# werner-duvaud/muzero-general

Measured on NVIDIA H100. Metric: self-play env-steps/sec, higher is better.
Workload: dtype f32 nets + f64 tree statistics

## Files before the change

muzero_general_b200/csrc/fc_search.cu:

```cuda
#include "fc_net.cuh"
#include "tree.cuh"
#include "kernels.h"

#include <stdlib.h>
#include <algorithm>
#include <vector>

namespace mz {

struct GameSmem {
    int vsum, mval, root_prior, visit, expansion, reward, prior, path, path_reward, hidden, act, bytes;
};

__host__ __device__ inline GameSmem game_smem_layout(int N, int A, int E, int maxw, bool keep_hidden) {
    GameSmem L;
    const int S = (N + 1) * A;
    const int Epad = (E + 3) & ~3;
    int off = 0;
    auto take = [&](int bytes) { int o = off; off = (off + bytes + 15) & ~15; return o; };
    L.vsum = take(S * 8);
    L.mval = take(S * 8);
    L.root_prior = take(A * 8);
    L.visit = take(S * 4);
    L.expansion = take(S * 4);
    L.reward = take(S * 4);
    L.prior = take(S * 4);
    L.path = take((N + 2) * 4);
    L.path_reward = take((N + 2) * 4);
    L.hidden = take((keep_hidden ? (N + 1) * Epad : 0) * 4);
    L.act = take(9 * maxw * 4);
    off += 16;
    L.bytes = off;
    return L;
}

enum { kPhRoot, kPhSelect, kPhNet, kPhExpand, kPhBackup, kPhLevels, kPhRounds, kPhSims, kPhSums,
       kPhStart = kPhSums, kPhEnd, kPhCount };
#ifdef MZ_FC_PHASES
constexpr int kPhMaxGames = 1 << 16;
__device__ unsigned long long g_fc_phase[kPhMaxGames][kPhCount];
MZ_DEVINL unsigned long long global_ns() {
    unsigned long long t;
    asm volatile("mov.u64 %0, %%globaltimer;" : "=l"(t));
    return t;
}
struct PhaseClock {
    int row = -1;
    unsigned last = 0;
    MZ_DEVINL void start(int g, bool leader) {
        row = (leader && g < kPhMaxGames) ? g : -1;
        if (row >= 0) atomicExch(&g_fc_phase[row][kPhStart], global_ns());
        last = (unsigned)clock();
    }
    MZ_DEVINL void finish() { if (row >= 0) atomicExch(&g_fc_phase[row][kPhEnd], global_ns()); }
    MZ_DEVINL void mark(int p) {
        const unsigned now = (unsigned)clock();
        if (row >= 0) atomicAdd(&g_fc_phase[row][p], (unsigned long long)(now - last));
        last = now;
    }
    MZ_DEVINL void count(int p, int n) { if (row >= 0) atomicAdd(&g_fc_phase[row][p], (unsigned long long)n); }
};
#else
struct PhaseClock {
    MZ_DEVINL void start(int, bool) {}
    MZ_DEVINL void finish() {}
    MZ_DEVINL void mark(int) {}
    MZ_DEVINL void count(int, int) {}
};
#endif

enum { kTapRaw, kTapReward, kTapPolicy, kTapValue };
struct NoTap { MZ_DEVINL void operator()(int, const float*, int) const {} };

template <int G, typename Tap>
MZ_DEVINL void fc_root_inference(const FcNet& net, const float* blob, const float* obs, float* hidden, float* s0, float* s1,
                                 float* s2, int E, int S, int A, float& logit, float& value, Tap&& tap) {
    const int lane = LaneGroup<G>::lane();
    load_vector<G>(obs, s1, net.obs_elems);
    float* raw = mlp_forward<G>(net.rep, blob, s1, s0, s1, s2);
    tap(kTapRaw, raw, E);
    rescale_unit_range<G>(raw, hidden, E);
    float* pol = mlp_forward<G>(net.pol, blob, hidden, s0, s1, s2);
    logit = (lane < A) ? pol[lane] : 0.0f;
    tap(kTapPolicy, pol, A);
    LaneGroup<G>::sync();
    float* val = mlp_forward<G>(net.val, blob, hidden, s0, s1, s2);
    value = support_to_scalar_group<G>(val, S);
    tap(kTapValue, val, 2 * S + 1);
    LaneGroup<G>::sync();
}

template <int G, typename SH, typename Tap>
MZ_DEVINL void fc_sim_inference(const FcNet& net, const float* blob, const float* h, int action, float* hn, float* s0, float* s1,
                                float* s2, float* const (&hb)[3][2], bool fused_heads, int E, int S, int A, float& logit,
                                float& prior, float& value, float& reward, Tap&& tap) {
    const int lane = LaneGroup<G>::lane();
    const int F = 2 * S + 1;
    if constexpr (SH::kEnabled) {
        fc_recurrent_fixed<G, SH>(net, blob, h, action, hn, s0, s1, hb[0][0], hb[1][0], hb[2][0], prior, value, reward);
        tap(kTapRaw, s1, E);
    } else {
        float* raw = mlp_forward<G>(net.dyn, blob, h, s0, s1, s2, action);
        if (fused_heads) {
            rescale_unit_range<G>(raw, hn, E);
            const MlpDesc* const ds[3] = {&net.rew, &net.pol, &net.val};
            const float* const xs[3] = {raw, hn, hn};
            float* outs[3];
            mlp_forward_multi<G, 3>(ds, blob, xs, hb, outs);
            logit = (lane < A) ? outs[1][lane] : 0.0f;
            support_to_scalar_group2<G>(outs[2], outs[0], S, value, reward);
            tap(kTapRaw, raw, E); tap(kTapReward, outs[0], F); tap(kTapPolicy, outs[1], A); tap(kTapValue, outs[2], F);
            LaneGroup<G>::sync();
        } else {
            float* rl = mlp_forward<G>(net.rew, blob, raw, s0, s1, nullptr);
            reward = support_to_scalar_group<G>(rl, S);
            tap(kTapRaw, raw, E); tap(kTapReward, rl, F);
            LaneGroup<G>::sync();
            rescale_unit_range<G>(raw, hn, E);
            float* pol = mlp_forward<G>(net.pol, blob, hn, s0, s1, s2);
            logit = (lane < A) ? pol[lane] : 0.0f;
            tap(kTapPolicy, pol, A);
            LaneGroup<G>::sync();
            float* vl = mlp_forward<G>(net.val, blob, hn, s0, s1, s2);
            value = support_to_scalar_group<G>(vl, S);
            tap(kTapValue, vl, F);
            LaneGroup<G>::sync();
        }
        prior = group_softmax_masked<G>(logit, lane < A);
    }
}

template <typename SH>
constexpr int fixed_actions() {
    if constexpr (SH::kEnabled) return SH::A;
    else return 0;
}

template <int G, bool kTeacher, typename SH, int kP>
__global__ void __launch_bounds__(kFcMaxThreads, 2) fc_search_kernel(const __grid_constant__ FcSearchArgs a) {
    extern __shared__ __align__(16) unsigned char smem[];
    constexpr int kA = fixed_actions<SH>();
    const int N = a.N, A = kA ? kA : a.A;
    double* s_pbc = reinterpret_cast<double*>(smem);
    double* s_sqrt = s_pbc + (N + 2);
    float* s_blob = reinterpret_cast<float*>(s_sqrt + (N + 2));
    for (int i = threadIdx.x; i < N + 2; i += blockDim.x) { s_pbc[i] = a.pbc[i]; s_sqrt[i] = a.sqrtn[i]; }
    if (!kTeacher)
        for (int i = threadIdx.x; i < a.net.blob_floats; i += blockDim.x) s_blob[i] = a.blob[i];
    __syncthreads();

    const int shared_bytes = ((2 * (N + 2) * 8 + (kTeacher ? 0 : a.net.blob_floats) * 4) + 15) & ~15;
    const GameSmem L = game_smem_layout(N, A, a.net.E, a.net.maxw, !kTeacher);
    const int groups_per_cta = blockDim.x / G;
    const int gi = threadIdx.x / G;
    const int lane = LaneGroup<G>::lane();
    unsigned char* mine = smem + shared_bytes + (size_t)gi * L.bytes;

    TreeConst c;
    c.A = A; c.N = N; c.P = a.P; c.discount = a.discount; c.noise_frac = a.noise_frac; c.noise_alpha = a.noise_alpha; c.seed = a.seed;
    c.pbc = s_pbc; c.sqrtn = s_sqrt; c.ucb = a.ucb;

    GameTree t;
    t.vsum = reinterpret_cast<double*>(mine + L.vsum);
    t.mval = reinterpret_cast<double*>(mine + L.mval);
    t.root_prior = reinterpret_cast<double*>(mine + L.root_prior);
    t.visit = reinterpret_cast<int*>(mine + L.visit);
    t.expansion = reinterpret_cast<int*>(mine + L.expansion);
    t.reward = reinterpret_cast<float*>(mine + L.reward);
    t.prior = reinterpret_cast<float*>(mine + L.prior);
    t.path = reinterpret_cast<int*>(mine + L.path);
    t.path_reward = reinterpret_cast<float*>(mine + L.path_reward);
    float* s_hidden = reinterpret_cast<float*>(mine + L.hidden);
    float* s_act = reinterpret_cast<float*>(mine + L.act);
    const int E = a.net.E, S = a.net.S, maxw = a.net.maxw;
    const int Epad = (E + 3) & ~3;
    float* s0 = s_act;
    float* s1 = s_act + maxw;
    float* s2 = s_act + 2 * maxw;
    float* const hb[3][2] = {{s_act + 3 * maxw, s_act + 4 * maxw}, {s_act + 5 * maxw, s_act + 6 * maxw},
                             {s_act + 7 * maxw, s_act + 8 * maxw}};
    const bool fused_heads = (a.net.rew.n == a.net.pol.n) && (a.net.pol.n == a.net.val.n);
    constexpr int kMaxD = select_levels_for(kA ? kA : 2, G);
    const SelectLanes sl = select_lanes<G, kA>(A, min(a.select_levels, kMaxD));
    PhaseClock ph;

    const int warp_first = (int)blockIdx.x * groups_per_cta + (int)(threadIdx.x & ~31u) / G;
    for (int g0 = warp_first; g0 < a.n_games; g0 += gridDim.x * groups_per_cta) {
        const int g_own = g0 + gi - (int)(threadIdx.x & ~31u) / G;
        const bool own = g_own < a.n_games;
        const int g = own ? g_own : a.n_games - 1;
        ph.start(g, lane == 0 && own);
        const int64_t game_id = a.game_id ? a.game_id[g] : (int64_t)g;
        const int move = a.move_index ? a.move_index[g] : 0;
        const int to_play0 = a.to_play ? a.to_play[g] : 0;
        const int first_index = a.first_index ? a.first_index[g] : -1;
        unsigned legal = 0;
        for (int k = 0; k < A; ++k) legal |= (a.legal_mask == nullptr || a.legal_mask[(size_t)g * A + k]) ? (1u << k) : 0u;
        t.legal = legal;
        (void)to_play0;

        float root_value, root_reward, logit = 0.0f;
        if (kTeacher) {
            root_value = a.teacher.root_value[g];
            root_reward = a.teacher.root_reward[g];
        } else {
            fc_root_inference<G>(a.net, s_blob, a.obs + (size_t)g * a.net.obs_elems, s_hidden, s0, s1, s2, E, S, A, logit, root_value,
                                 NoTap{});
            root_reward = inverse_value_transform(0.0f);
        }
        float prior;
        if (kTeacher) prior = (lane < A) ? a.teacher.root_priors[(size_t)g * A + lane] : 0.0f;
        else prior = group_softmax_masked<G>(logit, lane < A && ((legal >> lane) & 1u));
        if (a.trace.root_priors_raw && lane < A && own) a.trace.root_priors_raw[(size_t)g * A + lane] = ((legal >> lane) & 1u) ? prior : 0.0f;
        if (a.trace.root_reward && lane == 0 && own) a.trace.root_reward[g] = root_reward;
        tree_init_root<G, kA>(c, t, prior, root_reward,
                              (a.add_noise && a.noise) ? a.noise + (size_t)g * A : nullptr, a.add_noise && !a.noise,
                              game_id, move, (a.trace.noise && own) ? a.trace.noise + (size_t)g * A : nullptr);
        ph.mark(kPhRoot);

        int max_depth = 0;
        LaneGroup<G>::converge();
        for (int sim = 0; sim < N; ++sim) {
            int rounds;
            const Leaf leaf = tree_select_lookahead<G, kMaxD, kA>(c, t, sl, sim, game_id, move, first_index, rounds);
            ph.mark(kPhSelect);
            ph.count(kPhLevels, leaf.depth);
            ph.count(kPhRounds, rounds);
            float value, reward;
            if (kTeacher) {
                value = a.teacher.value[(size_t)g * N + sim];
                reward = a.teacher.reward[(size_t)g * N + sim];
                prior = (lane < A) ? a.teacher.priors[((size_t)g * N + sim) * A + lane] : 0.0f;
            } else {
                fc_sim_inference<G, SH>(a.net, s_blob, s_hidden + (size_t)leaf.parent_exp * Epad, leaf.action,
                                        s_hidden + (size_t)t.n_expanded * Epad, s0, s1, s2, hb, fused_heads, E, S, A, logit, prior, value, reward,
                                        NoTap{});
            }
            ph.mark(kPhNet);
            if (a.trace.depth && own) {
                const size_t ti = (size_t)g * N + sim;
                if (lane == 0) { a.trace.depth[ti] = leaf.depth; a.trace.value[ti] = value; a.trace.reward[ti] = reward; }
                if (lane < A) a.trace.priors[ti * A + lane] = prior;
                for (int j = lane; j < leaf.depth && j < a.trace.max_depth; j += G)
                    a.trace.actions[ti * a.trace.max_depth + j] = (uint8_t)(t.path[j + 1] % A);
            }
            tree_expand<G, kA>(c, t, leaf, reward, prior);
            ph.mark(kPhExpand);
            tree_backup<G, kP, true>(c, t, leaf, value);
            ph.mark(kPhBackup);
            max_depth = max(max_depth, leaf.depth);
        }
        ph.count(kPhSims, N);

        if (lane < A && own) {
            const bool ok = (legal >> lane) & 1u;
            if (a.visit_counts) a.visit_counts[(size_t)g * A + lane] = ok ? t.visit[lane] : 0;
            if (a.root_priors) a.root_priors[(size_t)g * A + lane] = t.root_prior[lane];
        }
        if (lane == 0 && own) {
            if (a.root_value) a.root_value[g] = (t.root_visit == 0) ? 0.0 : __ddiv_rn(t.root_vsum, (double)t.root_visit);
            if (a.root_predicted_value) a.root_predicted_value[g] = root_value;
            if (a.max_tree_depth) a.max_tree_depth[g] = max_depth;
            if (a.tie_count) a.tie_count[g] = t.ties;
            if (a.value_range) { a.value_range[2 * g] = t.lo; a.value_range[2 * g + 1] = t.hi; }
        }
        if (a.pool.visit && own) {
            const int slots = (N + 1) * A;
            const size_t pb = (size_t)g * slots;
            for (int s = lane; s < t.n_expanded * A; s += G) {
                a.pool.visit[pb + s] = t.visit[s];
                a.pool.vsum[pb + s] = t.vsum[s];
                a.pool.reward[pb + s] = t.reward[s];
                a.pool.prior[pb + s] = t.prior[s];
                a.pool.expansion[pb + s] = t.expansion[s];
            }
            if (lane < A) a.pool.root_prior[(size_t)g * A + lane] = t.root_prior[lane];
            if (!kTeacher && a.pool.hidden)
                for (int i = lane; i < t.n_expanded * E; i += G)
                    a.pool.hidden[(size_t)g * (N + 1) * E + i] = s_hidden[(i / E) * Epad + (i % E)];
            if (lane == 0) {
                a.pool.root_visit[g] = t.root_visit;
                a.pool.root_vsum[g] = t.root_vsum;
                a.pool.n_expanded[g] = t.n_expanded;
            }
        }
        ph.finish();
        LaneGroup<G>::sync();
    }
}

static size_t fc_cta_smem(int N, int A, int E, int maxw, int blob_floats, bool teacher, int groups) {
    const GameSmem L = game_smem_layout(N, A, E, maxw, !teacher);
    const size_t shared_bytes = ((2 * (size_t)(N + 2) * 8 + (teacher ? 0 : (size_t)blob_floats) * 4) + 15) & ~(size_t)15;
    return shared_bytes + (size_t)groups * L.bytes;
}

bool fc_search_plan(int N, int A, int E, int maxw, int blob_floats, int G, bool teacher, int n_games, int sm_count,
                    size_t smem_per_sm, size_t smem_reserve, size_t smem_cap, int regs, int threads, FcPlan* plan) {
    if (n_games < 1 || sm_count < 1 || G < 1 || regs < 1 || N < 0 || A < 1 || E < 1 || maxw < 1 || blob_floats < 0) return false;
    bool found = false;
    const std::vector<int> sizes = threads != 0 ? std::vector<int>{threads} : std::vector<int>{64, 128, 256};
    for (int t : sizes) {
        if (t % 32 != 0 || t < G || t > kFcMaxThreads) continue;
        const int groups = t / G;
        const size_t smem = fc_cta_smem(N, A, E, maxw, blob_floats, teacher, groups);
        const int by_smem = smem > smem_cap ? 0 : (int)(smem_per_sm / ((smem + smem_reserve + 127) & ~(size_t)127));
        const int by_regs = (65536 / (((regs * 32) + 255) & ~255)) / (t / 32);
        const int per_sm = std::min(std::min(by_smem, by_regs), std::min(2048 / t, 32));
        if (per_sm >= 1) {
            const int slots = per_sm * groups * sm_count;
            const int passes = (n_games + slots - 1) / slots;
            if (!found || passes < plan->passes) {
                *plan = FcPlan{t, groups, per_sm, slots, passes, smem};
                found = true;
            }
        }
    }
    return found;
}

template <int G, bool T, typename SH, int kP>
static cudaError_t launch_kernel(const FcSearchArgs& a, const FcLaunchInfo& l, cudaStream_t stream) {
    fc_search_kernel<G, T, SH, kP><<<l.grid, l.block, l.smem, stream>>>(a);
    return cudaGetLastError();
}

template <int G, bool T, typename SH, int kP = 0>
static cudaError_t prepare_one(const FcSearchArgs& a, bool one_level, int sm_count, FcLaunchState* st, FcPrepared* p) {
    p->select_levels = one_level ? 1 : select_levels_for(a.A, G);
    auto kern = fc_search_kernel<G, T, SH, kP>;
    const void* fn = reinterpret_cast<const void*>(kern);
    int regs = 0;
    for (const auto& k : st->kernels) if (k.fn == fn) regs = k.regs;
    if (regs == 0) {
        cudaError_t err = cudaFuncSetAttribute(kern, cudaFuncAttributeMaxDynamicSharedMemorySize, (int)st->smem_cap);
        if (err == cudaSuccess) err = cudaFuncSetAttribute(kern, cudaFuncAttributePreferredSharedMemoryCarveout, cudaSharedmemCarveoutMaxShared);
        cudaFuncAttributes fa{};
        if (err == cudaSuccess) err = cudaFuncGetAttributes(&fa, kern);
        if (err != cudaSuccess) return err;
        regs = fa.numRegs;
        st->kernels.push_back({fn, regs});
    }
    FcPlan plan;
    if (!fc_search_plan(a.N, a.A, a.net.E, a.net.maxw, a.net.blob_floats, G, T, a.n_games, sm_count, st->smem_per_sm,
                        st->smem_reserve, st->smem_cap, regs, a.threads, &plan))
        return cudaErrorInvalidConfiguration;
    int per_sm = -1;
    for (const auto& s : st->shapes) if (s.fn == fn && s.threads == plan.threads && s.smem == plan.smem) per_sm = s.ctas_per_sm;
    if (per_sm < 0) {
        cudaError_t err = cudaOccupancyMaxActiveBlocksPerMultiprocessor(&per_sm, kern, plan.threads, plan.smem);
        if (err != cudaSuccess) return err;
        st->shapes.push_back({fn, plan.threads, plan.smem, per_sm});
    }
    per_sm = std::min(per_sm, plan.ctas_per_sm);
    if (per_sm < 1) return cudaErrorInvalidConfiguration;
    const int want = (a.n_games + plan.groups - 1) / plan.groups;
    const int grid = std::min(want, per_sm * sm_count);
    p->launch = launch_kernel<G, T, SH, kP>;
    p->fixed_shape = SH::kEnabled;
    p->info = FcLaunchInfo{grid, plan.threads, per_sm, G, plan.smem};
    return cudaSuccess;
}

using CartPoleShape = FcFixedShape<8, 16, 10, 2>;

static bool fc_uses_fixed(const FcNet& net, int G) { return (G == 16 || G == 32) && fc_matches_fixed<CartPoleShape>(net); }

static cudaError_t prepare_fc_search(const FcSearchArgs& a, int group, bool teacher, bool generic, bool one_level,
                                     int sm_count, FcLaunchState* st, FcPrepared* p) {
    if (!teacher && !generic && fc_uses_fixed(a.net, group)) {
        if (group == 16 && a.P == 1) return prepare_one<16, false, CartPoleShape, 1>(a, one_level, sm_count, st, p);
        if (group == 16) return prepare_one<16, false, CartPoleShape>(a, one_level, sm_count, st, p);
        if (group == 32 && a.P == 1) return prepare_one<32, false, CartPoleShape, 1>(a, one_level, sm_count, st, p);
        if (group == 32) return prepare_one<32, false, CartPoleShape>(a, one_level, sm_count, st, p);
    }
#define MZ_CASE(GG)                                                                                     \
    case GG:                                                                                            \
        return teacher ? prepare_one<GG, true, FcGenericShape>(a, one_level, sm_count, st, p)           \
                       : prepare_one<GG, false, FcGenericShape>(a, one_level, sm_count, st, p);
    switch (group) {
        MZ_CASE(4)
        MZ_CASE(8)
        MZ_CASE(16)
        MZ_CASE(32)
    }
#undef MZ_CASE
    return cudaErrorInvalidValue;
}

cudaError_t launch_fc_search(const FcSearchArgs& a_in, int group, bool teacher, int sm_count, FcLaunchState* st,
                             cudaStream_t stream) {
    const char* generic = getenv("MZ_FC_GENERIC");
    const char* levels = getenv("MZ_FC_SELECT_LEVELS");
    FcPreparedKey key{a_in.n_games, group, a_in.threads, teacher, generic && generic[0] == '1',
                      levels && levels[0] == '1' && levels[1] == 0};
    FcPrepared& p = st->prepared;
    if (!p.valid || !(p.key == key)) {
        p.valid = false;
        const cudaError_t err = prepare_fc_search(a_in, group, teacher, key.generic, key.one_level, sm_count, st, &p);
        if (err != cudaSuccess) return err;
        p.key = key;
        p.valid = true;
    }
    FcSearchArgs a = a_in;
    a.select_levels = p.select_levels;
    const cudaError_t err = p.launch(a, p.info, stream);
    if (err == cudaSuccess) {
        st->launched = true;
        st->last = p.info;
    }
    return err;
}

struct CopyTap {
    const FcDebugArgs* a;
    int g, lane, step;
    bool own;
    MZ_DEVINL void operator()(int what, const float* v, int n) const {
        float* dst = what == kTapRaw ? a->raw : what == kTapReward ? a->reward_logits : what == kTapPolicy ? a->policy_logits : a->value_logits;
        if (!dst || !own) return;
        for (int i = lane; i < n; i += step) dst[(size_t)g * n + i] = v[i];
    }
};

template <int G, typename SH>
__global__ void __launch_bounds__(32) fc_debug_net_kernel(const __grid_constant__ FcDebugArgs a) {
    extern __shared__ __align__(16) unsigned char smem[];
    float* s_blob = reinterpret_cast<float*>(smem);
    for (int i = threadIdx.x; i < a.net.blob_floats; i += blockDim.x) s_blob[i] = a.blob[i];
    __syncthreads();
    const int E = a.net.E, A = a.net.A, maxw = a.net.maxw, Epad = (E + 3) & ~3;
    const GameSmem L = game_smem_layout(1, A, E, maxw, true);
    const int groups_per_cta = blockDim.x / G;
    const int gi = threadIdx.x / G;
    const int lane = LaneGroup<G>::lane();
    unsigned char* mine = smem + ((a.net.blob_floats * 4 + 15) & ~15) + (size_t)gi * L.bytes;
    float* s_hidden = reinterpret_cast<float*>(mine + L.hidden);
    float* s_act = reinterpret_cast<float*>(mine + L.act);
    float* s0 = s_act;
    float* s1 = s_act + maxw;
    float* s2 = s_act + 2 * maxw;
    float* const hb[3][2] = {{s_act + 3 * maxw, s_act + 4 * maxw}, {s_act + 5 * maxw, s_act + 6 * maxw},
                             {s_act + 7 * maxw, s_act + 8 * maxw}};
    const bool fused_heads = (a.net.rew.n == a.net.pol.n) && (a.net.pol.n == a.net.val.n) && !a.force_split;
    const int warp_first = (int)blockIdx.x * groups_per_cta + (int)(threadIdx.x & ~31u) / G;
    for (int g0 = warp_first; g0 < a.n; g0 += gridDim.x * groups_per_cta) {
        const int g_own = g0 + gi - (int)(threadIdx.x & ~31u) / G;
        const bool own = g_own < a.n;
        const int g = own ? g_own : a.n - 1;
        for (int i = lane; i < L.bytes / 4; i += G) reinterpret_cast<unsigned*>(mine)[i] = 0xFFFFFFFFu;
        LaneGroup<G>::sync();
        const CopyTap tap{&a, g, lane, G, own};
        float logit = 0.0f, prior, value, reward = 0.0f;
        float* hn = s_hidden;
        if (a.route == MZ_FC_SEARCH_ROOT) {
            fc_root_inference<G>(a.net, s_blob, a.in + (size_t)g * a.net.obs_elems, s_hidden, s0, s1, s2, E, a.net.S, A, logit, value,
                                 tap);
            prior = group_softmax_masked<G>(logit, lane < A);
        } else {
            load_vector<G>(a.in + (size_t)g * E, s_hidden, E);
            hn = s_hidden + Epad;
            fc_sim_inference<G, SH>(a.net, s_blob, s_hidden, a.action[g], hn, s0, s1, s2, hb, fused_heads, E, a.net.S, A, logit, prior, value,
                                    reward, tap);
        }
        if (own) {
            if (a.hidden) for (int i = lane; i < E; i += G) a.hidden[(size_t)g * E + i] = hn[i];
            if (a.prior && lane < A) a.prior[(size_t)g * A + lane] = prior;
            if (lane == 0) {
                if (a.value) a.value[g] = value;
                if (a.reward && a.route == MZ_FC_SEARCH_SIM) a.reward[g] = reward;
            }
        }
        LaneGroup<G>::sync();
    }
}

bool fc_debug_plan(const FcNet& net, int G, int route, bool force_split, int n, int sm_count, size_t smem_cap, int64_t* plan,
                   std::string* err) {
    if (G != 4 && G != 8 && G != 16 && G != 32) { *err = "the lane group must be 4, 8, 16 or 32"; return false; }
    if (n < 1 || sm_count < 1) { *err = "bad batch or SM count"; return false; }
    if (route == MZ_FC_INFER_INITIAL || route == MZ_FC_INFER_RECURRENT || route == MZ_FC_INFER_POOL) {
        FcInferPlan p;
        if (!fc_infer_plan(net.blob_floats, net.maxw, G, n, sm_count, smem_cap, &p)) {
            *err = "fc_inference_kernel needs " + std::to_string(fc_infer_smem(net.blob_floats, net.maxw, 32 / G)) +
                   " bytes of shared memory for one warp, the device allows " + std::to_string(smem_cap);
            return false;
        }
        const int64_t out[5] = {MZ_FC_PATH_INFER, G, p.threads, p.grid, (int64_t)p.smem};
        for (int i = 0; i < 5; ++i) plan[i] = out[i];
        return true;
    }
    if (route != MZ_FC_SEARCH_ROOT && route != MZ_FC_SEARCH_SIM) { *err = "unknown route"; return false; }
    if (net.A > G) { *err = "the search needs one lane per action (action_space <= lane group)"; return false; }
    const bool fixed = fc_uses_fixed(net, G) && !force_split;
    const bool fused = net.rew.n == net.pol.n && net.pol.n == net.val.n && !force_split;
    const GameSmem L = game_smem_layout(1, net.A, net.E, net.maxw, true);
    const size_t smem = (size_t)((net.blob_floats * 4 + 15) & ~15) + (size_t)(32 / G) * L.bytes;
    if (smem > smem_cap) {
        *err = "the search's network call needs " + std::to_string(smem) + " bytes of shared memory, the device allows " +
               std::to_string(smem_cap);
        return false;
    }
    const int groups = 32 / G;
    const int grid = std::min((n + groups - 1) / groups, 8 * sm_count);
    const int64_t out[5] = {fixed ? MZ_FC_PATH_FIXED : fused ? MZ_FC_PATH_FUSED : MZ_FC_PATH_SPLIT, G, 32, grid, (int64_t)smem};
    for (int i = 0; i < 5; ++i) plan[i] = out[i];
    return true;
}

template <int G, typename SH>
static cudaError_t launch_debug(const FcDebugArgs& a, int grid, size_t smem, cudaStream_t stream) {
    auto kern = fc_debug_net_kernel<G, SH>;
    cudaError_t err = cudaFuncSetAttribute(kern, cudaFuncAttributeMaxDynamicSharedMemorySize, (int)smem);
    if (err != cudaSuccess) return err;
    kern<<<grid, 32, smem, stream>>>(a);
    return cudaGetLastError();
}

cudaError_t launch_fc_debug_net(const FcDebugArgs& a, int G, const int64_t* plan, cudaStream_t stream) {
    const int grid = (int)plan[3];
    const size_t smem = (size_t)plan[4];
    if (plan[0] == MZ_FC_PATH_FIXED) {
        if (G == 16) return launch_debug<16, CartPoleShape>(a, grid, smem, stream);
        if (G == 32) return launch_debug<32, CartPoleShape>(a, grid, smem, stream);
        return cudaErrorInvalidValue;
    }
    switch (G) {
        case 4: return launch_debug<4, FcGenericShape>(a, grid, smem, stream);
        case 8: return launch_debug<8, FcGenericShape>(a, grid, smem, stream);
        case 16: return launch_debug<16, FcGenericShape>(a, grid, smem, stream);
        case 32: return launch_debug<32, FcGenericShape>(a, grid, smem, stream);
    }
    return cudaErrorInvalidValue;
}

#ifdef MZ_FC_PHASES
extern "C" int mz_fc_phase_counters(unsigned long long* out, int reset) {
    cudaError_t e = cudaDeviceSynchronize();
    void* dev = nullptr;
    if (e == cudaSuccess) e = cudaGetSymbolAddress(&dev, g_fc_phase);
    if (e == cudaSuccess && out) {
        std::vector<unsigned long long> rows((size_t)kPhMaxGames * kPhCount);
        e = cudaMemcpy(rows.data(), dev, rows.size() * 8, cudaMemcpyDeviceToHost);
        for (int p = 0; p < kPhSums; ++p) out[p] = 0;
        for (size_t i = 0; i < rows.size(); ++i) if (i % kPhCount < kPhSums) out[i % kPhCount] += rows[i];
    }
    if (e == cudaSuccess && reset) e = cudaMemset(dev, 0, sizeof(g_fc_phase));
    if (e == cudaSuccess) e = cudaDeviceSynchronize();
    return e == cudaSuccess ? 0 : (int)e;
}

extern "C" int mz_fc_phase_spans(unsigned long long* out, int n) {
    if (!out || n < 0 || n > kPhMaxGames) return (int)cudaErrorInvalidValue;
    std::vector<unsigned long long> rows((size_t)n * kPhCount);
    cudaError_t e = cudaDeviceSynchronize();
    if (e == cudaSuccess) e = cudaMemcpyFromSymbol(rows.data(), g_fc_phase, rows.size() * 8);
    for (int g = 0; e == cudaSuccess && g < n; ++g) {
        out[2 * g] = rows[(size_t)g * kPhCount + kPhStart];
        out[2 * g + 1] = rows[(size_t)g * kPhCount + kPhEnd];
    }
    return e == cudaSuccess ? 0 : (int)e;
}
#endif

}
```

muzero_general_b200/engine.py:

```python
from __future__ import annotations

import ctypes as C
import math
from dataclasses import dataclass
from typing import Optional

import numpy

from . import _lib
from .netspec import FC, NetSpec, netspec_from_config, weights_spec


def _is_torch(x):
    return x is not None and type(x).__module__.startswith("torch")


def _fill_layers(desc, prefix, layers):
    if len(layers) > _lib.MZ_MAX_LAYERS:
        raise ValueError(f"at most {_lib.MZ_MAX_LAYERS} hidden layers per head are supported")
    setattr(desc, "n_" + prefix, len(layers))
    arr = getattr(desc, prefix)
    for i, v in enumerate(layers):
        arr[i] = int(v)


def net_desc(spec: NetSpec) -> _lib.MzNetDesc:
    d = _lib.MzNetDesc()
    d.kind = spec.kind
    d.obs_c, d.obs_h, d.obs_w = spec.in_channels, spec.obs_shape[1], spec.obs_shape[2]
    d.action_space = spec.action_space
    d.support_size = spec.support_size
    d.encoding = spec.encoding
    _fill_layers(d, "fc_representation", spec.fc_representation)
    _fill_layers(d, "fc_dynamics", spec.fc_dynamics)
    _fill_layers(d, "fc_reward", spec.fc_reward)
    _fill_layers(d, "fc_value", spec.fc_value)
    _fill_layers(d, "fc_policy", spec.fc_policy)
    d.blocks, d.channels = spec.blocks, spec.channels
    d.reduced_reward, d.reduced_value, d.reduced_policy = spec.reduced_reward, spec.reduced_value, spec.reduced_policy
    _fill_layers(d, "res_fc_reward", spec.res_fc_reward)
    _fill_layers(d, "res_fc_value", spec.res_fc_value)
    _fill_layers(d, "res_fc_policy", spec.res_fc_policy)
    d.downsample = spec.downsample
    return d


@dataclass
class SearchOutput:
    visit_counts: numpy.ndarray
    root_value: numpy.ndarray
    root_predicted_value: numpy.ndarray
    max_tree_depth: numpy.ndarray
    tie_count: numpy.ndarray
    root_priors: numpy.ndarray
    value_range: numpy.ndarray
    trace: Optional[dict] = None
    device_ms: float = 0.0


_OUT_FIELDS = (("int32", -1), ("float64", 0), ("float32", 0), ("int32", 0), ("int32", 0), ("float64", -1), ("float64", 2))


def output_layout(n, A):
    fields, off = [], 0
    for dt, cols in _OUT_FIELDS:
        shape = (n,) if cols == 0 else (n, A if cols < 0 else cols)
        fields.append((dt, shape, (1,) if cols == 0 else (shape[1], 1), off))
        off += (numpy.dtype(dt).itemsize * math.prod(shape) + 15) & ~15
    return tuple(fields), off


def carve_outputs(buf, fields):
    import torch
    views = {"float64": buf, "float32": buf.view(torch.float32), "int32": buf.view(torch.int32)}
    return SearchOutput(*[views[dt].as_strided(shape, strides, off // (8 if dt == "float64" else 4))
                          for dt, shape, strides, off in fields])


_TORCH_DTYPES = {}


class SearchEngine:
    def __init__(self, config, max_games: int = 1, device: int = 0, seed: Optional[int] = None,
                 num_simulations: Optional[int] = None, extra_expansions: int = 0):
        self.lib = _lib.load_library()
        self.config = config
        self.spec = netspec_from_config(config)
        if list(config.action_space) != list(range(len(config.action_space))):
            raise ValueError("action_space must be list(range(n)) (every reference game file is)")
        if list(config.players) != list(range(len(config.players))):
            raise ValueError("players must be list(range(n))")
        self.A = self.spec.action_space
        self.N = int(config.num_simulations if num_simulations is None else num_simulations)
        self.max_games = int(max_games)
        self.device = int(device)
        self.extra_expansions = int(extra_expansions)
        self.pool_n = self.N + self.extra_expansions
        s = _lib.MzSearchDesc()
        s.max_games = self.max_games
        s.num_simulations = self.N
        s.extra_expansions = self.extra_expansions
        s.num_players = len(config.players)
        s.discount = float(config.discount)
        s.pb_c_base = float(config.pb_c_base)
        s.pb_c_init = float(config.pb_c_init)
        s.root_dirichlet_alpha = float(config.root_dirichlet_alpha)
        s.root_exploration_fraction = float(config.root_exploration_fraction)
        s.seed = int(config.seed if seed is None else seed) & 0xFFFFFFFFFFFFFFFF
        n = self.pool_n + 2
        self._pbc = (C.c_double * n)(*[math.log((i + config.pb_c_base + 1) / config.pb_c_base) + config.pb_c_init
                                       for i in range(n)])
        self._sqrt = (C.c_double * n)(*[math.sqrt(i) for i in range(n)])
        s.pb_c_table = C.cast(self._pbc, C.POINTER(C.c_double))
        s.sqrt_table = C.cast(self._sqrt, C.POINTER(C.c_double))
        self._ucb = (C.c_double * (n * n))(*[self._pbc[p] * (self._sqrt[p] / (c + 1)) for p in range(n) for c in range(n)])
        s.ucb_table = C.cast(self._ucb, C.POINTER(C.c_double))
        self._net_desc = net_desc(self.spec)
        handle = C.c_void_p()
        rc = self.lib.mz_create(C.byref(self._net_desc), C.byref(s), self.device, C.byref(handle))
        if rc != 0:
            msg = self.lib.mz_last_error(None).decode()
            if rc == _lib.MZ_EUNSUPPORTED:
                raise NotImplementedError(msg)
            raise _lib.MzError(rc, msg)
        self._h = handle
        self.hidden_elems = int(self.lib.mz_hidden_elems(self._h))
        self.obs_elems = int(self.lib.mz_obs_elems(self._h))
        self._dio = _lib.MzDeviceSearchIO()
        self._dio_ref = C.byref(self._dio)
        self._layouts = {}

    def close(self):
        if getattr(self, "_h", None):
            self.lib.mz_destroy(self._h)
            self._h = None

    def __del__(self):
        try:
            self.close()
        except Exception:
            pass

    def _check(self, rc):
        if rc != 0:
            raise _lib.MzError(rc, self.lib.mz_last_error(self._h).decode())

    @property
    def launch_count(self):
        return int(self.lib.mz_launch_count(self._h))

    @property
    def graph_partitions(self):
        return int(self.lib.mz_graph_partitions(self._h))

    @property
    def last_fc_launch(self):
        info = (C.c_int64 * 5)()
        if self.lib.mz_fc_last_launch(self._h, info) != 1:
            return None
        return dict(zip(("grid", "block", "group", "smem", "ctas_per_sm"), (int(v) for v in info)))

    @property
    def fc_prepared(self):
        info = (C.c_int64 * 7)()
        if self.lib.mz_debug_fc_prepared(self._h, info) != 1:
            return None
        return dict(zip(("games", "group", "threads", "generic", "one_level", "select_levels", "fixed_shape"),
                        (int(v) for v in info)))

    @property
    def last_search_ms(self):
        return float(self.lib.mz_last_search_ms(self._h))

    @property
    def numerics(self):
        return self.lib.mz_numerics(self._h).decode()

    KERNEL_CLASSES = ("tree_step_kernel", "conv_tower_tc_kernel", "heads_kernel", "conv3x3_kernel", "other", "small_tower_kernel",
                      "small_search_kernel")

    def kernel_timing(self, enable):
        self._check(self.lib.mz_kernel_timing(self._h, 1 if enable else 0))

    def kernel_times(self):
        import ctypes as C
        ms = (C.c_double * len(self.KERNEL_CLASSES))()
        cnt = (C.c_int64 * len(self.KERNEL_CLASSES))()
        self._check(self.lib.mz_kernel_times(self._h, ms, cnt))
        return {k: (float(ms[i]), int(cnt[i])) for i, k in enumerate(self.KERNEL_CLASSES)}

    @staticmethod
    def _ptr(x, dtype, keep):
        if x is None:
            return None
        if _is_torch(x):
            if not _TORCH_DTYPES:
                import torch
                _TORCH_DTYPES.update({numpy.float32: torch.float32, numpy.float64: torch.float64, numpy.int32: torch.int32,
                                      numpy.int64: torch.int64, numpy.uint8: torch.uint8})
            want = _TORCH_DTYPES[dtype]
            if x.dtype != want or not x.is_contiguous():
                x = x.to(want).contiguous()
            keep.append(x)
            return x.data_ptr()
        a = numpy.ascontiguousarray(x, dtype=dtype)
        keep.append(a)
        return a.ctypes.data

    def load_weights(self, state_dict):
        tensors, keep = [], []
        for key, shape in weights_spec(self.spec):
            if key.endswith("num_batches_tracked"):
                continue
            if key not in state_dict:
                raise KeyError(f"state_dict is missing {key}")
            v = state_dict[key]
            if _is_torch(v):
                v = v.detach().cpu().numpy()
            a = numpy.ascontiguousarray(v, dtype=numpy.float32)
            if tuple(a.shape) != tuple(shape):
                raise ValueError(f"{key}: expected shape {tuple(shape)}, got {tuple(a.shape)}")
            keep.append(a)
            tensors.append((key.encode(), a))
        arr = (_lib.MzTensor * len(tensors))()
        for i, (name, a) in enumerate(tensors):
            arr[i].name = name
            arr[i].data = a.ctypes.data
            arr[i].numel = a.size
        self._check(self.lib.mz_load_weights(self._h, arr, len(tensors)))

    def search(self, obs=None, legal_mask=None, to_play=None, add_exploration_noise=False, noise=None,
               first_index=None, game_id=None, move_index=None, teacher=None, trace=False, trace_depth=None,
               keep_tree=False, stepwise=False, n_games=None, continue_tree=False) -> SearchOutput:
        A, N = self.A, self.N
        keep = []
        if n_games is None:
            src = obs if obs is not None else (teacher["root_value"] if teacher else legal_mask)
            n_games = 1 if (src is None and continue_tree) else int(src.shape[0])
        n = n_games
        device_mem = _is_torch(obs)
        if legal_mask is not None and not _is_torch(legal_mask):
            assert numpy.asarray(legal_mask).reshape(n, -1).any(axis=1).all(), \
                "Legal actions should not be an empty array."
        if device_mem and teacher is None and not (trace or keep_tree or stepwise or continue_tree):
            return self._search_device(n, obs, legal_mask, to_play, add_exploration_noise, noise, first_index, game_id,
                                       move_index)
        io = _lib.MzSearchIO()
        io.n_games = n
        io.mem = _lib.MZ_MEM_DEVICE if device_mem else _lib.MZ_MEM_HOST
        if obs is not None:
            if not device_mem:
                obs = numpy.asarray(obs, dtype=numpy.float32).reshape(n, -1)
                if obs.shape[1] != self.obs_elems:
                    raise ValueError(f"observation has {obs.shape[1]} elements, expected {self.obs_elems}")
            io.obs = self._ptr(obs, numpy.float32, keep)
        io.legal_mask = self._ptr(legal_mask, numpy.uint8, keep)
        io.to_play = self._ptr(to_play, numpy.int32, keep)
        io.add_exploration_noise = int(bool(add_exploration_noise))
        io.flags = ((_lib.MZ_FLAG_KEEP_TREE if keep_tree else 0) | (_lib.MZ_FLAG_STEPWISE if stepwise else 0)
                    | (_lib.MZ_FLAG_CONTINUE if continue_tree else 0))
        io.noise = self._ptr(noise, numpy.float64, keep)
        io.first_index = self._ptr(first_index, numpy.int32, keep)
        io.game_id = self._ptr(game_id, numpy.int64, keep)
        io.move_index = self._ptr(move_index, numpy.int32, keep)

        if device_mem:
            import torch
            dev = obs.device
            mk = lambda shape, dt: torch.empty(shape, dtype=dt, device=dev)
            out = SearchOutput(mk((n, A), torch.int32), mk((n,), torch.float64), mk((n,), torch.float32),
                               mk((n,), torch.int32), mk((n,), torch.int32), mk((n, A), torch.float64),
                               mk((n, 2), torch.float64))
            p = lambda t: t.data_ptr()
        else:
            out = SearchOutput(numpy.empty((n, A), numpy.int32), numpy.empty(n, numpy.float64),
                               numpy.empty(n, numpy.float32), numpy.empty(n, numpy.int32), numpy.empty(n, numpy.int32),
                               numpy.empty((n, A), numpy.float64), numpy.empty((n, 2), numpy.float64))
            p = lambda a: a.ctypes.data
        io.visit_counts, io.root_value, io.root_predicted_value = p(out.visit_counts), p(out.root_value), p(out.root_predicted_value)
        io.max_tree_depth, io.tie_count, io.root_priors = p(out.max_tree_depth), p(out.tie_count), p(out.root_priors)
        io.value_range = p(out.value_range)

        if teacher is not None:
            t = _lib.MzTeacher()
            for f in ("root_value", "root_reward", "root_priors", "value", "reward", "priors"):
                setattr(t, f, self._ptr(teacher[f], numpy.float32, keep))
            keep.append(t)
            io.teacher = C.pointer(t)
        if trace:
            if device_mem:
                raise ValueError("trace is only available with host buffers")
            D = int(trace_depth or max(1, N))
            tr = dict(depth=numpy.zeros((n, N), numpy.int32), actions=numpy.zeros((n, N, D), numpy.uint8),
                      value=numpy.zeros((n, N), numpy.float32), reward=numpy.zeros((n, N), numpy.float32),
                      priors=numpy.zeros((n, N, A), numpy.float32), root_priors_raw=numpy.zeros((n, A), numpy.float32),
                      root_reward=numpy.zeros(n, numpy.float32), noise=numpy.zeros((n, A), numpy.float64))
            t = _lib.MzTrace()
            t.max_depth = D
            for k, v in tr.items():
                setattr(t, k, v.ctypes.data)
            keep.append(t)
            io.trace = C.pointer(t)
            out.trace = tr
        self._check(self.lib.mz_search(self._h, C.byref(io)))
        out.device_ms = self.last_search_ms
        return out

    def _search_device(self, n, obs, legal_mask, to_play, add_noise, noise, first_index, game_id, move_index):
        import torch
        keep, io = [], self._dio
        io.n_games = n
        io.add_exploration_noise = 1 if add_noise else 0
        io.obs = self._ptr(obs, numpy.float32, keep)
        io.noise = self._ptr(noise, numpy.float64, keep)
        io.game_id = self._ptr(game_id, numpy.int64, keep)
        io.move_index = self._ptr(move_index, numpy.int32, keep)
        io.legal_mask = self._ptr(legal_mask, numpy.uint8, keep)
        io.to_play = self._ptr(to_play, numpy.int32, keep)
        io.first_index = self._ptr(first_index, numpy.int32, keep)
        layout = self._layouts.get(n)
        if layout is None:
            layout = self._layouts[n] = output_layout(n, self.A)
        fields, nbytes = layout
        buf = torch.empty(nbytes // 8, dtype=torch.float64, device=obs.device)
        base = buf.data_ptr()
        (io.visit_counts, io.root_value, io.root_predicted_value, io.max_tree_depth, io.tie_count, io.root_priors,
         io.value_range) = (base + f[3] for f in fields)
        self._check(self.lib.mz_search_device(self._h, self._dio_ref))
        try:
            out = carve_outputs(buf, fields)
        finally:
            self._check(self.lib.mz_search_device_wait(self._h, self._dio_ref))
        out.device_ms = io.device_ms
        return out

    def _inference(self, fn, n, x, action):
        A, F, H = self.A, self.spec.full_support, self.hidden_elems
        keep = []
        res = dict(value_logits=numpy.empty((n, F), numpy.float32), reward_logits=numpy.empty((n, F), numpy.float32),
                   policy_logits=numpy.empty((n, A), numpy.float32), hidden=numpy.empty((n, H), numpy.float32),
                   value=numpy.empty(n, numpy.float32), reward=numpy.empty(n, numpy.float32))
        o = _lib.MzInferenceOut()
        for k, v in res.items():
            setattr(o, k, v.ctypes.data)
        xp = self._ptr(numpy.asarray(x, dtype=numpy.float32).reshape(n, -1), numpy.float32, keep)
        if action is None:
            self._check(fn(self._h, n, _lib.MZ_MEM_HOST, xp, C.byref(o)))
        else:
            ap = self._ptr(numpy.asarray(action).reshape(n), numpy.int32, keep)
            self._check(fn(self._h, n, _lib.MZ_MEM_HOST, xp, ap, C.byref(o)))
        return res

    def initial_inference(self, obs):
        obs = numpy.asarray(obs, dtype=numpy.float32)
        return self._inference(self.lib.mz_initial_inference, obs.shape[0], obs, None)

    def recurrent_inference(self, hidden, action):
        hidden = numpy.asarray(hidden, dtype=numpy.float32)
        return self._inference(self.lib.mz_recurrent_inference, hidden.shape[0], hidden, action)

    def _reanalyse_io(self, frames, frame_offsets, actions, action_offsets, positions, stacked_observations, keep):
        device_mem = _is_torch(frames)
        if not device_mem:
            frames = numpy.asarray(frames, dtype=numpy.float32)
        O = int(frames.shape[1]) if frames.ndim == 2 else int(numpy.prod(tuple(frames.shape[1:]), dtype=numpy.int64))
        io = _lib.MzReanalyseIO()
        positions = numpy.ascontiguousarray(positions, dtype=numpy.int64)
        io.n_games = len(positions)
        io.mem = _lib.MZ_MEM_DEVICE if device_mem else _lib.MZ_MEM_HOST
        io.stacked_observations = int(self.config.stacked_observations if stacked_observations is None
                                      else stacked_observations)
        io.frame_elems = O
        io.frames = self._ptr(frames, numpy.float32, keep)
        io.actions = self._ptr(actions, numpy.int32, keep)
        io.frame_offsets = self._ptr(numpy.asarray(frame_offsets, dtype=numpy.int64), numpy.int64, keep)
        io.action_offsets = self._ptr(numpy.asarray(action_offsets, dtype=numpy.int64), numpy.int64, keep)
        io.positions = self._ptr(positions, numpy.int64, keep)
        return io, int(positions.sum()), device_mem

    def reanalyse_values(self, frames, frame_offsets, actions, action_offsets, positions, stacked_observations=None):
        keep = []
        io, total, device_mem = self._reanalyse_io(frames, frame_offsets, actions, action_offsets, positions,
                                                   stacked_observations, keep)
        if device_mem:
            import torch
            values = torch.empty(total, dtype=torch.float32, device=frames.device)
            io.values = values.data_ptr() if total else None
        else:
            values = numpy.empty(total, numpy.float32)
            io.values = values.ctypes.data if total else None
        self._check(self.lib.mz_reanalyse_values(self._h, C.byref(io)))
        return values

    def reanalyse_search(self, frames, frame_offsets, actions, action_offsets, positions, legal_mask=None, to_play=None,
                         game_id=None, add_exploration_noise=True, stacked_observations=None):
        keep = []
        io, total, device_mem = self._reanalyse_io(frames, frame_offsets, actions, action_offsets, positions,
                                                   stacked_observations, keep)
        if device_mem:
            import torch
            to_dev = lambda x, dt: x if x is None or _is_torch(x) else torch.as_tensor(numpy.asarray(x, dt), device=frames.device)
            legal_mask, to_play = to_dev(legal_mask, numpy.uint8), to_dev(to_play, numpy.int32)
        sio = _lib.MzReanalyseSearchIO()
        sio.games = C.addressof(io)
        sio.legal_mask = self._ptr(legal_mask, numpy.uint8, keep)
        sio.to_play = self._ptr(to_play, numpy.int32, keep)
        sio.game_id = self._ptr(None if game_id is None else numpy.asarray(game_id, dtype=numpy.int64).reshape(-1),
                                numpy.int64, keep)
        sio.add_exploration_noise = int(bool(add_exploration_noise))
        if device_mem:
            visits = torch.empty((total, self.A), dtype=torch.int32, device=frames.device)
            root = torch.empty(total, dtype=torch.float64, device=frames.device)
            p = lambda t: t.data_ptr() if total else None
        else:
            visits = numpy.empty((total, self.A), numpy.int32)
            root = numpy.empty(total, numpy.float64)
            p = lambda a: a.ctypes.data if total else None
        sio.visit_counts, sio.root_value = p(visits), p(root)
        self._check(self.lib.mz_reanalyse_search(self._h, C.byref(sio)))
        return visits, root

    def debug_reanalyse_stack(self, chunk, frames, frame_offsets, actions, action_offsets, positions,
                              stacked_observations=None):
        keep = []
        io, total, _ = self._reanalyse_io(frames, frame_offsets, actions, action_offsets, positions, stacked_observations,
                                          keep)
        n = max(0, min(self.max_games, total - int(chunk) * self.max_games))
        out = numpy.empty((n, self.obs_elems), numpy.float32)
        self._check(self.lib.mz_debug_reanalyse_stack(self._h, C.byref(io), int(chunk), out.ctypes.data if n else None))
        return out

    def export_tree(self, game: int, with_hidden: bool = False):
        S = (self.pool_n + 1) * self.A
        out = dict(child_visit=numpy.zeros(S, numpy.int32), child_value_sum=numpy.zeros(S, numpy.float64),
                   child_reward=numpy.zeros(S, numpy.float32), child_prior=numpy.zeros(S, numpy.float64),
                   child_expansion=numpy.full(S, -1, numpy.int32))
        e = _lib.MzTreeExport()
        for k, v in out.items():
            setattr(e, k, v.ctypes.data)
        if with_hidden:
            out["hidden"] = numpy.zeros((self.pool_n + 1, self.hidden_elems), numpy.float32)
            e.hidden = out["hidden"].ctypes.data
        self._check(self.lib.mz_export_tree(self._h, int(game), C.byref(e)))
        out["n_expansions"] = int(e.n_expansions)
        out["root_visit"] = int(e.root_visit)
        out["root_value_sum"] = float(e.root_value_sum)
        out["root_reward"] = float(e.root_reward)
        return out

    def import_tree(self, game: int, tree: dict):
        keep = []
        K = int(tree["n_expansions"])
        e = _lib.MzTreeExport()
        e.n_expansions = K
        for k, dt in (("child_visit", numpy.int32), ("child_value_sum", numpy.float64), ("child_reward", numpy.float32),
                      ("child_prior", numpy.float64), ("child_expansion", numpy.int32)):
            a = numpy.ascontiguousarray(tree[k], dtype=dt).reshape(-1)
            assert a.size >= K * self.A, k
            keep.append(a)
            setattr(e, k, a.ctypes.data)
        if tree.get("hidden") is not None:
            hdn = numpy.ascontiguousarray(tree["hidden"], dtype=numpy.float32).reshape(-1)
            assert hdn.size >= K * self.hidden_elems
            keep.append(hdn)
            e.hidden = hdn.ctypes.data
        e.root_visit = int(tree["root_visit"])
        e.root_value_sum = float(tree["root_value_sum"])
        e.root_reward = float(tree.get("root_reward", 0.0))
        self._check(self.lib.mz_import_tree(self._h, int(game), C.byref(e)))


class DeviceSelfPlayLoop:

    ENVS = {"cartpole": _lib.MZ_ENV_CARTPOLE, "tictactoe": _lib.MZ_ENV_TICTACTOE, "connect4": _lib.MZ_ENV_CONNECT4,
            "gomoku": _lib.MZ_ENV_GOMOKU, "twentyone": _lib.MZ_ENV_TWENTYONE, "simple_grid": _lib.MZ_ENV_SIMPLE_GRID,
            "gridworld": _lib.MZ_ENV_GRIDWORLD}
    OPPONENTS = {"self": _lib.MZ_OPPONENT_SELF, "expert": _lib.MZ_OPPONENT_EXPERT, "random": _lib.MZ_OPPONENT_RANDOM}

    def __init__(self, engine: SearchEngine, env: str, max_moves: int, temperature_threshold=None, reward_scale: int = 1,
                 first_game_id: int = 0, staging_bytes: int = 0, game_id_stride: int = 0, td_steps: int = 0,
                 per_alpha: float = 1.0, discount: float = 1.0, opponent: str = "self", muzero_player: int = 0,
                 stacked_observations: int = 0):
        if env not in self.ENVS:
            raise NotImplementedError(f"no device-resident environment for {env!r}")
        if opponent not in self.OPPONENTS:
            raise NotImplementedError(f"no device opponent {opponent!r} (expected one of {sorted(self.OPPONENTS)})")
        self.engine = engine
        self.opponent, self.muzero_player = opponent, int(muzero_player)
        d = self._desc(self.ENVS[env], max_moves, temperature_threshold, reward_scale, first_game_id, staging_bytes,
                       game_id_stride, td_steps, per_alpha, discount, stacked_observations)
        try:
            engine._check(engine.lib.mz_selfplay_begin_vs(engine._h, C.byref(d), self.OPPONENTS[opponent], self.muzero_player))
        except _lib.MzError as e:
            if e.code == _lib.MZ_EUNSUPPORTED:
                raise NotImplementedError(str(e)) from e
            raise
        self.stats = _lib.MzSelfPlayStats()

    def _desc(self, env, max_moves, temperature_threshold, reward_scale, first_game_id, staging_bytes, game_id_stride,
              td_steps, per_alpha, discount, stacked_observations):
        d = _lib.MzSelfPlayDesc()
        d.env = env
        d.max_moves = int(max_moves)
        d.temperature_threshold = int(temperature_threshold or 0)
        d.reward_scale = int(reward_scale)
        d.first_game_id = int(first_game_id)
        d.game_id_stride = int(game_id_stride)
        d.stacked_observations = int(stacked_observations)
        if td_steps and per_alpha in (0.5, 1, 1.0):
            self._discount_pow = (C.c_double * (int(td_steps) + 1))(*[discount ** k for k in range(int(td_steps) + 1)])
            d.td_steps, d.per_alpha = int(td_steps), float(per_alpha)
            d.discount_pow = C.cast(self._discount_pow, C.c_void_p)
        self.with_priorities = bool(d.td_steps)
        d.staging_bytes = int(staging_bytes)
        return d

    def _inject(self, keep, forced_action, uniform, noise, first_index):
        if forced_action is None and uniform is None and noise is None and first_index is None:
            return None
        eng = self.engine
        inj = _lib.MzSelfPlayInject()
        inj.forced_action = eng._ptr(forced_action, numpy.int32, keep)
        inj.uniform = eng._ptr(uniform, numpy.float64, keep)
        inj.noise = eng._ptr(noise, numpy.float64, keep)
        inj.first_index = eng._ptr(first_index, numpy.int32, keep)
        return inj

    def moves(self, n_moves: int, temperature: float, forced_action=None, uniform=None, noise=None, first_index=None):
        eng = self.engine
        keep = []
        inj = self._inject(keep, forced_action, uniform, noise, first_index)
        eng._check(eng.lib.mz_selfplay_moves(eng._h, int(n_moves), float(temperature),
                                            C.byref(inj) if inj is not None else None, C.byref(self.stats)))
        return self.stats

    def enqueue(self, n_moves: int, temperature: float):
        eng = self.engine
        eng._check(eng.lib.mz_selfplay_enqueue(eng._h, int(n_moves), float(temperature)))

    def wait(self):
        eng = self.engine
        eng._check(eng.lib.mz_selfplay_wait(eng._h, C.byref(self.stats)))
        return self.stats

    def drain_pointers(self):
        eng = self.engine
        ptr, nbytes, ngames, iptr = C.c_void_p(), C.c_uint64(), C.c_int32(), C.c_void_p()
        eng._check(eng.lib.mz_selfplay_drain(eng._h, C.byref(ptr), C.byref(nbytes), C.byref(ngames), C.byref(iptr)))
        return ptr.value, int(nbytes.value), int(ngames.value), iptr.value

    @staticmethod
    def copy_staged(pointers):
        ptr, nbytes, n, iptr = pointers
        if n == 0:
            return b"", numpy.zeros((0, 2), numpy.uint64)
        index = numpy.frombuffer(C.string_at(iptr, 16 * n), numpy.uint64).reshape(n, 2)
        return C.string_at(ptr, nbytes), index

    def drain(self):
        return self.copy_staged(self.drain_pointers())

    def peek(self):
        eng = self.engine
        B, A = eng.max_games, eng.A
        out = dict(obs=numpy.empty((B, eng.obs_elems), numpy.float32), legal_mask=numpy.empty((B, A), numpy.uint8),
                   to_play=numpy.empty(B, numpy.int32), game_id=numpy.empty(B, numpy.int64),
                   move_index=numpy.empty(B, numpy.int32), last_action=numpy.empty(B, numpy.int32))
        pk = _lib.MzSelfPlayPeek()
        for k, v in out.items():
            setattr(pk, k, v.ctypes.data)
        eng._check(eng.lib.mz_selfplay_peek(eng._h, C.byref(pk)))
        return out


class HostEnvSelfPlayLoop(DeviceSelfPlayLoop):

    OBS_HISTORIES = ("device", "host")

    def __init__(self, engine: SearchEngine, obs_shape, max_moves: int, obs, legal_mask, to_play,
                 temperature_threshold=None, first_game_id: int = 0, staging_bytes: int = 0, game_id_stride: int = 0,
                 td_steps: int = 0, per_alpha: float = 1.0, discount: float = 1.0, stacked_observations: int = 0,
                 obs_history: str = "device", opponent: str = "self", muzero_player: int = 0):
        if obs_history not in self.OBS_HISTORIES:
            raise ValueError(f"obs_history must be one of {self.OBS_HISTORIES}, got {obs_history!r}")
        if opponent not in self.OPPONENTS:
            raise NotImplementedError(f"no device opponent {opponent!r} (expected one of {sorted(self.OPPONENTS)})")
        self.engine = engine
        self.opponent, self.muzero_player = opponent, int(muzero_player)
        B = engine.max_games
        self.O = int(numpy.prod(obs_shape))
        d = self._desc(_lib.MZ_ENV_HOST, max_moves, temperature_threshold, 0, first_game_id, staging_bytes, game_id_stride,
                       td_steps, per_alpha, discount, stacked_observations)
        e = _lib.MzHostEnvDesc(*(int(x) for x in obs_shape))
        o, lg, tp = self._rows(obs, legal_mask, to_play)
        if opponent == "self" and self.muzero_player == 0:
            begin = engine.lib.mz_selfplay_begin_host if obs_history == "device" else engine.lib.mz_selfplay_begin_host_window
            engine._check(begin(engine._h, C.byref(d), C.byref(e), o.ctypes.data, lg.ctypes.data, tp.ctypes.data))
        else:
            rc = engine.lib.mz_selfplay_begin_host_vs(engine._h, C.byref(d), C.byref(e), self.OPPONENTS[opponent],
                                                      self.muzero_player, int(obs_history == "host"), o.ctypes.data,
                                                      lg.ctypes.data, tp.ctypes.data)
            if rc == _lib.MZ_EUNSUPPORTED:
                raise NotImplementedError(engine.lib.mz_last_error(engine._h).decode())
            engine._check(rc)
        self.obs_history = obs_history
        self.stats = _lib.MzSelfPlayStats()
        self.actions = numpy.empty(B, numpy.int32)
        self.finished = numpy.empty(B, numpy.uint8)
        self.defaults = numpy.empty(B, numpy.int32)
        if obs_history == "host":
            self._game_id = [int(first_game_id) + g for g in range(B)]
            self._stride = int(game_id_stride) if int(game_id_stride) > 0 else B
            self._rows_of = [[o[g].copy()] for g in range(B)]
            self._finished_rows = {}

    def _rows(self, obs, legal_mask, to_play):
        B = self.engine.max_games
        if not isinstance(obs, numpy.ndarray):
            obs = numpy.stack([numpy.asarray(x) for x in obs])
        return (numpy.ascontiguousarray(obs, numpy.float32).reshape(B, self.O),
                numpy.ascontiguousarray(legal_mask, numpy.uint8).reshape(B, self.engine.A),
                numpy.ascontiguousarray(to_play, numpy.int32).reshape(B))

    def act(self, temperature: float, forced_action=None, uniform=None, noise=None, first_index=None):
        eng = self.engine
        keep = []
        inj = self._inject(keep, forced_action, uniform, noise, first_index)
        eng._check(eng.lib.mz_selfplay_host_act(eng._h, float(temperature), C.byref(inj) if inj is not None else None,
                                               self.actions.ctypes.data))
        return self.actions

    def opponent_turn(self):
        eng = self.engine
# ... 371 lines not shown
```

Before: 13.68 million.

## Stage CTA prologue with cp.async, prefetch observations, preallocate next output buffer

The kernel prologue now copies the UCB tables and network weight blob into shared memory with cp.async (16-byte chunks for the blob) instead of plain per-thread loads, and prefetches each game's observation row into L1. On the host, the next call's output buffer is allocated with empty_like while the kernel runs, taking allocation off the critical path. Extra SM-id and CTA-entry timestamp instrumentation is added under the phase-profiling macro. The 16-byte blob copies round the float count up to a multiple of four and assume aligned source and destination.

```diff
diff --git a/muzero_general_b200/csrc/fc_search.cu b/muzero_general_b200/csrc/fc_search.cu
--- a/muzero_general_b200/csrc/fc_search.cu
+++ b/muzero_general_b200/csrc/fc_search.cu
@@ -35,7 +35,7 @@
 }
 
 enum { kPhRoot, kPhSelect, kPhNet, kPhExpand, kPhBackup, kPhLevels, kPhRounds, kPhSims, kPhSums,
-       kPhStart = kPhSums, kPhEnd, kPhCount };
+       kPhStart = kPhSums, kPhEnd, kPhSm, kPhCount };
 #ifdef MZ_FC_PHASES
 constexpr int kPhMaxGames = 1 << 16;
 __device__ unsigned long long g_fc_phase[kPhMaxGames][kPhCount];
@@ -52,7 +52,13 @@
         if (row >= 0) atomicExch(&g_fc_phase[row][kPhStart], global_ns());
         last = (unsigned)clock();
     }
-    MZ_DEVINL void finish() { if (row >= 0) atomicExch(&g_fc_phase[row][kPhEnd], global_ns()); }
+    MZ_DEVINL void finish() {
+        if (row < 0) return;
+        unsigned sm;
+        asm volatile("mov.u32 %0, %%smid;" : "=r"(sm));
+        atomicExch(&g_fc_phase[row][kPhEnd], global_ns());
+        atomicExch(&g_fc_phase[row][kPhSm], (unsigned long long)sm);
+    }
     MZ_DEVINL void mark(int p) {
         const unsigned now = (unsigned)clock();
         if (row >= 0) atomicAdd(&g_fc_phase[row][p], (unsigned long long)(now - last));
@@ -60,6 +66,9 @@
     }
     MZ_DEVINL void count(int p, int n) { if (row >= 0) atomicAdd(&g_fc_phase[row][p], (unsigned long long)n); }
 };
+constexpr int kPhMaxCtas = 1 << 14;
+__device__ unsigned long long g_fc_cta_entry[kPhMaxCtas];
+MZ_DEVINL void phase_cta_entry() { if (threadIdx.x == 0 && blockIdx.x < kPhMaxCtas) g_fc_cta_entry[blockIdx.x] = global_ns(); }
 #else
 struct PhaseClock {
     MZ_DEVINL void start(int, bool) {}
@@ -67,6 +76,7 @@
     MZ_DEVINL void mark(int) {}
     MZ_DEVINL void count(int, int) {}
 };
+MZ_DEVINL void phase_cta_entry() {}
 #endif
 
 enum { kTapRaw, kTapReward, kTapPolicy, kTapValue };
@@ -130,6 +140,14 @@
     }
 }
 
+MZ_DEVINL void cp_async8(void* dst, const void* src) {
+    asm volatile("cp.async.ca.shared.global [%0], [%1], 8;" ::"r"((unsigned)__cvta_generic_to_shared(dst)), "l"(src) : "memory");
+}
+MZ_DEVINL void cp_async16(void* dst, const void* src) {
+    asm volatile("cp.async.cg.shared.global [%0], [%1], 16;" ::"r"((unsigned)__cvta_generic_to_shared(dst)), "l"(src) : "memory");
+}
+MZ_DEVINL void cp_async_wait_all() { asm volatile("cp.async.wait_all;" ::: "memory"); }
+
 template <typename SH>
 constexpr int fixed_actions() {
     if constexpr (SH::kEnabled) return SH::A;
@@ -144,9 +162,15 @@
     double* s_pbc = reinterpret_cast<double*>(smem);
     double* s_sqrt = s_pbc + (N + 2);
     float* s_blob = reinterpret_cast<float*>(s_sqrt + (N + 2));
-    for (int i = threadIdx.x; i < N + 2; i += blockDim.x) { s_pbc[i] = a.pbc[i]; s_sqrt[i] = a.sqrtn[i]; }
+    phase_cta_entry();
+    if (!kTeacher && (threadIdx.x & (G - 1)) == 0) {
+        const int g = min((int)blockIdx.x * (int)(blockDim.x / G) + (int)threadIdx.x / G, a.n_games - 1);
+        asm volatile("prefetch.global.L1 [%0];" ::"l"(a.obs + (size_t)g * a.net.obs_elems));
+    }
+    for (int i = threadIdx.x; i < N + 2; i += blockDim.x) { cp_async8(s_pbc + i, a.pbc + i); cp_async8(s_sqrt + i, a.sqrtn + i); }
     if (!kTeacher)
-        for (int i = threadIdx.x; i < a.net.blob_floats; i += blockDim.x) s_blob[i] = a.blob[i];
+        for (int i = threadIdx.x; i < (a.net.blob_floats + 3) >> 2; i += blockDim.x) cp_async16(s_blob + 4 * i, a.blob + 4 * i);
+    cp_async_wait_all();
     __syncthreads();
 
     const int shared_bytes = ((2 * (N + 2) * 8 + (kTeacher ? 0 : a.net.blob_floats) * 4) + 15) & ~15;
@@ -561,6 +585,20 @@
     }
     return e == cudaSuccess ? 0 : (int)e;
 }
+
+extern "C" int mz_fc_phase_rows(unsigned long long* out, int n, int cols) {
+    if (!out || n < 0 || n > kPhMaxGames || cols != kPhCount) return (int)cudaErrorInvalidValue;
+    cudaError_t e = cudaDeviceSynchronize();
+    if (e == cudaSuccess) e = cudaMemcpyFromSymbol(out, g_fc_phase, (size_t)n * kPhCount * 8);
+    return e == cudaSuccess ? 0 : (int)e;
+}
+
+extern "C" int mz_fc_phase_ctas(unsigned long long* out, int n) {
+    if (!out || n < 0 || n > kPhMaxCtas) return (int)cudaErrorInvalidValue;
+    cudaError_t e = cudaDeviceSynchronize();
+    if (e == cudaSuccess) e = cudaMemcpyFromSymbol(out, g_fc_cta_entry, (size_t)n * 8);
+    return e == cudaSuccess ? 0 : (int)e;
+}
 #endif
 
 }
diff --git a/muzero_general_b200/engine.py b/muzero_general_b200/engine.py
--- a/muzero_general_b200/engine.py
+++ b/muzero_general_b200/engine.py
@@ -128,9 +128,10 @@
         self.obs_elems = int(self.lib.mz_obs_elems(self._h))
         self._dio = _lib.MzDeviceSearchIO()
         self._dio_ref = C.byref(self._dio)
-        self._layouts = {}
+        self._next_out = None
 
     def close(self):
+        self._next_out = None
         if getattr(self, "_h", None):
             self.lib.mz_destroy(self._h)
             self._h = None
@@ -318,17 +319,21 @@
         io.legal_mask = self._ptr(legal_mask, numpy.uint8, keep)
         io.to_play = self._ptr(to_play, numpy.int32, keep)
         io.first_index = self._ptr(first_index, numpy.int32, keep)
-        layout = self._layouts.get(n)
-        if layout is None:
-            layout = self._layouts[n] = output_layout(n, self.A)
-        fields, nbytes = layout
-        buf = torch.empty(nbytes // 8, dtype=torch.float64, device=obs.device)
+        key = (n, obs.get_device())
+        nxt, self._next_out = self._next_out, None
+        if nxt is not None and nxt[0] == key:
+            buf, fields, offsets = nxt[1]
+        else:
+            fields, nbytes = output_layout(n, self.A)
+            offsets = tuple(f[3] for f in fields)
+            buf = torch.empty(nbytes // 8, dtype=torch.float64, device=obs.device)
         base = buf.data_ptr()
         (io.visit_counts, io.root_value, io.root_predicted_value, io.max_tree_depth, io.tie_count, io.root_priors,
-         io.value_range) = (base + f[3] for f in fields)
+         io.value_range) = (base + o for o in offsets)
         self._check(self.lib.mz_search_device(self._h, self._dio_ref))
         try:
             out = carve_outputs(buf, fields)
+            self._next_out = (key, (torch.empty_like(buf), fields, offsets))
         finally:
             self._check(self.lib.mz_search_device_wait(self._h, self._dio_ref))
         out.device_ms = io.device_ms
```

Result: faster. 14.39 million, median of 6 (+5.1%).
